# dominikbuenger/torch_nfft

Measured on AMD Instinct MI355X. Metric: Mpoints/s (adjoint+forward, 3-D N=256 m=4), higher is better.
Workload: dtype f32

## Files before the change

### torch_nfft_amd/csrc/binning.hip

```cpp
#include <algorithm>
#include <hipcub/hipcub.hpp>

#include "common.h"
#include "kernels.h"
#include "range_items.h"

namespace nfft {

constexpr int kSortBlockPoints = 8192;
constexpr int kSortThreads = 512;
constexpr int kMaxPencilsLds = 8192;
constexpr int kSort2Parts = 8;

PlanLayout plan_layout(const Geom &g, int64_t n, int64_t B)
{
    PlanLayout L;
    L.cap = g.owned ? 4 * n : n;
    L.ntiles = (int64_t)g.tiles_per_batch * B * g.SB;
    L.npencils = (int64_t)g.nta[1] * g.nta[2] * B * g.l1seg;
    L.block_points = 1024;
    while (L.block_points < kSortBlockPoints &&
           (n > L.block_points * 512 || L.npencils * ((n + L.block_points - 1) / L.block_points) > (int64_t(1) << 20)))
        L.block_points *= 2;
    L.nblocks = (n + L.block_points - 1) / L.block_points;
    L.two_level = L.npencils <= kMaxPencilsLds && L.npencils * L.nblocks < (int64_t(1) << 28) && n > 0;
    const int64_t scan_items = L.two_level ? L.npencils * L.nblocks + 1 : L.ntiles + 1;
    L.scan_bytes = align_up(scan_items / 64 + 65536, 256);
    int64_t o = 0;
    L.off_offsets = o; o = align_up(o + (L.ntiles + 1) * 4, 256);
    L.off_cursor = o;  o = align_up(o + (L.ntiles + 1) * 4, 256);
    L.off_seal = o;    o += kSealBytes;
    L.off_perm = o;    o = align_up(o + (g.dim == 3 ? 0 : L.cap * 4), 256);
    L.off_spos = o;    o = align_up(o + L.cap * g.pstride * 4, 256);
    L.off_scan = o;    o = align_up(o + L.scan_bytes, 256);
    L.off_hist = o;    o = align_up(o + (L.two_level ? scan_items * 4 : 0), 256);
    L.off_hscan = o;   o = align_up(o + (L.two_level ? scan_items * 4 : 0), 256);
    L.off_tmp = o;     o = align_up(o + (L.two_level ? L.cap * 16 : 0), 256);
    L.off_hist2 = o;   o = align_up(o + (L.two_level ? L.npencils * kSort2Parts * (int64_t)g.l1bins * g.SB * g.CG * 4 : 0), 256);
    L.grouped = L.two_level && g.CG == 3;
    L.off_groups = o;  o = align_up(o + (L.grouped ? L.ntiles * 2 * 4 : 0), 256);
    L.work_cap = g.wide ? (int64_t)g.nta[1] * g.nta[2] * B * kSegMax + L.cap / 2048 + 16 : 0;
    L.work_head = 1 + (B * 8 + 15) / 16;
    L.off_work = o;    o = align_up(o + (g.wide ? (L.work_head + 2 * L.work_cap) * 16 : 0), 256);
    L.off_sealpart = o; o = align_up(o + (L.two_level ? L.nblocks * 8 : 0), 256);
    L.off_key1 = o;    o = align_up(o + (L.two_level && !g.owned ? n * 2 : 0), 256);
    L.off_key2 = o;    o = align_up(o + (L.two_level ? L.cap * 2 : 0), 256);
    L.total = o;
    return L;
}

__device__ __forceinline__ int point_tiles(const Geom &g, const float *__restrict__ pos, const int64_t *__restrict__ batch,
                                           int64_t i, int64_t B, int tiles[4])
{
    int cell[3] = {0, 0, 0};
    for (int u = 0; u < g.dim; ++u) {
        float fr;
        split_cell(pos[i * g.dim + u], g.M, cell[u + 3 - g.dim], fr);
    }
    int64_t b = batch ? batch[i] : 0;
    b = b < 0 ? 0 : (b >= B ? B - 1 : b);
    if (g.owned) {
        int pen[4];
        const int k = owned_pencils(g, cell[1], cell[2], pen);
        for (int q = 0; q < k; ++q) tiles[q] = (int)b * g.tiles_per_batch + pen[q] * g.np0 + cell[0];
        return k;
    }
    tiles[0] = ((int)b * g.tiles_per_batch + tile_of_cells(g, cell)) * g.SB + sub_of_cells(g, cell);
    return 1;
}

constexpr int kSealThreads = 1024;
// ... 121 lines not shown
    const int64_t hi = min(n, lo + block_points);
    unsigned long long seal = 0;
    for (int64_t i0 = lo + threadIdx.x; i0 < hi; i0 += (int64_t)kSortThreads * kSortUnroll) {
        float c0[kSortUnroll], c1[kSortUnroll], c2[kSortUnroll];
        int64_t bb[kSortUnroll];
#pragma unroll
        for (int q = 0; q < kSortUnroll; ++q) {
            const int64_t i = i0 + (int64_t)q * kSortThreads;
            const bool live = i < hi;
            load_point(pos, g.dim, i, live, c0[q], c1[q], c2[q]);
            bb[q] = live && batch ? batch[i] : 0;
        }
#pragma unroll
        for (int q = 0; q < kSortUnroll; ++q) {
            if (i0 + (int64_t)q * kSortThreads >= hi) continue;
            if (seal_part) seal += seal_point(g.dim, i0 + (int64_t)q * kSortThreads, c0[q], c1[q], c2[q], batch != nullptr, bb[q]);
            if (bb[q] < 0 || bb[q] >= B) report_fault(status, kFaultBatchIndex);
            const int64_t b = bb[q] < 0 ? 0 : (bb[q] >= B ? B - 1 : bb[q]);
            int bins[4];
            const int k = l1_bins_of(g, c0[q], c1[q], c2[q], b, bins);
            for (int r = 0; r < k; ++r) atomicAdd(&lds_hist[bins[r]], 1);
            if (!g.owned) key1[i0 + (int64_t)q * kSortThreads] = (unsigned short)bins[0];
        }
    }
    __syncthreads();
    for (int i = threadIdx.x; i < npencils; i += kSortThreads) hist[(int64_t)i * nblocks + blockIdx.x] = lds_hist[i];
    if (seal_part) {
        __shared__ unsigned long long part[16];
        seal = seal_block_sum(seal, part);
        if (threadIdx.x == 0) seal_part[blockIdx.x] = seal;
    }
}

template <bool COMMON>
__global__ void __launch_bounds__(kSortThreads)
sort1_scatter_kernel(Geom g_in, const float *__restrict__ pos, const int64_t *__restrict__ batch, int64_t n, int64_t B,
                     int npencils, int nblocks, int block_points, const int *__restrict__ hscan, const unsigned short *__restrict__ key1,
                     float4 *__restrict__ tmp, const unsigned long long *__restrict__ seal_part, unsigned long long *__restrict__ seal,
                     int *__restrict__ final_offsets, int *__restrict__ final_perm, float *__restrict__ final_spos,
                     const int *__restrict__ hist_raw)
{
    const bool final_pass = !COMMON && final_offsets != nullptr;
    const bool local_scan = final_pass && hist_raw != nullptr;
    if (final_pass && !local_scan && blockIdx.x == 0) {
        for (int i = threadIdx.x; i <= npencils; i += kSortThreads) final_offsets[i] = hscan[(int64_t)i * nblocks];
    }
    if (seal && blockIdx.x == 0) {
        __shared__ unsigned long long part[16];
        unsigned long long sum = 0;
        for (int i = threadIdx.x; i < nblocks; i += kSortThreads) sum += seal_part[i];
        sum = seal_block_sum(sum, part);
        if (threadIdx.x == 0) seal[0] = sum;
        if (threadIdx.x >= 1 && threadIdx.x < (int)(kSealBytes / 8)) seal[threadIdx.x] = 0ull;
        __syncthreads();
    }
    Geom g = g_in;
    if constexpr (COMMON) { g.dim = 3; g.owned = 0; }
    extern __shared__ int lds_cur[];
    if (local_scan) {
        int *const row = lds_cur + npencils;
        for (int i = threadIdx.x; i < npencils; i += kSortThreads) { lds_cur[i] = 0; row[i] = 0; }
        __syncthreads();
        int G = 1;
        while (2 * G * npencils <= kSortThreads && G < 64) G *= 2;
        const int sub = threadIdx.x & (G - 1);
        for (int p = threadIdx.x / G; p < npencils; p += kSortThreads / G) {
            int all = 0, before = 0;
            for (int bl = sub; bl < nblocks; bl += G) {
                const int c = hist_raw[p * nblocks + bl];
                all += c;
                before += bl < (int)blockIdx.x ? c : 0;
            }
            if (all) atomicAdd(&row[p], all);
            if (before) atomicAdd(&lds_cur[p], before);
        }
        __syncthreads();
        if (threadIdx.x < 64) {
            int carry = 0;
            for (int base = 0; base < npencils; base += 64) {
                const int idx = base + threadIdx.x;
                const int tot = idx < npencils ? row[idx] : 0;
                int incl = tot;
                for (int off = 1; off < 64; off <<= 1) {
                    const int t = __shfl_up(incl, off);
                    if ((int)threadIdx.x >= off) incl += t;
                }
                if (idx < npencils) {
                    const int excl = carry + incl - tot;
                    lds_cur[idx] += excl;
                    if (blockIdx.x == 0) final_offsets[idx] = excl;
// ... 10 lines not shown
    const int64_t hi = min(n, lo + block_points);
    for (int64_t i0 = lo + threadIdx.x; i0 < hi; i0 += (int64_t)kSortThreads * kSortUnroll) {
        float c0[kSortUnroll], c1[kSortUnroll], c2[kSortUnroll];
        int64_t bb[kSortUnroll];
        int kk[kSortUnroll];
#pragma unroll
        for (int q = 0; q < kSortUnroll; ++q) {
            const int64_t i = i0 + (int64_t)q * kSortThreads;
            const bool live = i < hi;
            load_point(pos, g.dim, i, live, c0[q], c1[q], c2[q]);
            bb[q] = live && batch && g.owned ? batch[i] : 0;
            kk[q] = live && !g.owned ? key1[i] : 0;
        }
#pragma unroll
        for (int q = 0; q < kSortUnroll; ++q) {
            const int64_t i = i0 + (int64_t)q * kSortThreads;
            if (i >= hi) continue;
            int bins[4];
            int k = 1;
            if (!g.owned) {
                bins[0] = kk[q];
            } else {
                const int64_t b = bb[q] < 0 ? 0 : (bb[q] >= B ? B - 1 : bb[q]);
                k = l1_bins_of(g, c0[q], c1[q], c2[q], b, bins);
            }
            for (int r = 0; r < k; ++r) {
                const int slot = atomicAdd(&lds_cur[bins[r]], 1);
                if (final_pass) {
                    final_perm[slot] = (int)i;
                    final_spos[(int64_t)slot * g.dim] = c0[q];
                    if (g.dim > 1) final_spos[(int64_t)slot * g.dim + 1] = c1[q];
                    continue;
                }
                tmp[slot] = make_float4(c0[q], c1[q], c2[q], __int_as_float((int)i));
            }
        }
    }
}

__device__ __forceinline__ int fine_key(const Geom &g, const float4 rec, const int bin_lo, const int col0)
{
    if (g.dim != 3) return 0;
    int cell[3];
    float fr;
    split_cell(rec.x, g.M, cell[0], fr);
    int key = (g.bin0 == 1 ? cell[0] : div_small(cell[0], g.bin0)) - bin_lo;
    if (g.SB > 1) {
        split_cell(rec.y, g.M, cell[1], fr);
        split_cell(rec.z, g.M, cell[2], fr);
        key = key * g.SB + sub_of_cells(g, cell);
    }
    if (g.CG > 1) {
        split_cell(rec.z, g.M, cell[2], fr);
        key = key * g.CG + column_group(cell[2] - col0, g.W);
    }
    return key;
}

__device__ __forceinline__ void sort2_range(const int *__restrict__ hscan, int l1, int nblocks, int part, int &p0,
                                            int &r0, int &r1)
{
    p0 = hscan[(int64_t)l1 * nblocks];
    const int p1 = hscan[(int64_t)(l1 + 1) * nblocks];
    const int64_t len = p1 - p0;
    r0 = p0 + (int)(len * part / kSort2Parts);
    r1 = p0 + (int)(len * (part + 1) / kSort2Parts);
}

template <bool COMMON>
__global__ void __launch_bounds__(kSortThreads)
sort2_count_kernel(Geom g_in, int nblocks, const int *__restrict__ hscan, const float4 *__restrict__ tmp,
                   int *__restrict__ hist2 , unsigned short *__restrict__ key2 )
{
    Geom g = g_in;
    if constexpr (COMMON) { g.dim = 3; g.owned = 0; }
    extern __shared__ int lds2[];
    const int l1 = blockIdx.x, part = blockIdx.y;
    const int pencil = l1 / g.l1seg, sg = l1 - pencil * g.l1seg;
    const int bin_lo = sg * g.l1bins;
    const int col0 = (pencil % g.nta[2]) * g.Ta[2];
    const int nt0 = (min(g.np0, bin_lo + g.l1bins) - bin_lo) * g.SB * g.CG;
    int p0, r0, r1;
    sort2_range(hscan, l1, nblocks, part, p0, r0, r1);
    for (int i = threadIdx.x; i < nt0; i += kSortThreads) lds2[i] = 0;
    __syncthreads();
    for (int j0 = r0 + threadIdx.x; j0 < r1; j0 += kSortThreads * 8) {
        float4 rec[8];
#pragma unroll
        for (int q = 0; q < 8; ++q) {
            const int j = j0 + q * kSortThreads;
            rec[q] = j < r1 ? tmp[j] : make_float4(0.f, 0.f, 0.f, 0.f);
        }
#pragma unroll
        for (int q = 0; q < 8; ++q)
            if (j0 + q * kSortThreads < r1) {
                const int key = fine_key(g, rec[q], bin_lo, col0);
                atomicAdd(&lds2[key], 1);
                key2[j0 + q * kSortThreads] = (unsigned short)key;
            }
    }
    __syncthreads();
    int *out = hist2 + ((int64_t)l1 * kSort2Parts + part) * g.l1bins * g.SB * g.CG;
    for (int i = threadIdx.x; i < nt0; i += kSortThreads) out[i] = lds2[i];
}

__global__ void __launch_bounds__(kSortThreads)
sort2_scatter_kernel(Geom g, int npencils, int nblocks, const int *__restrict__ hscan, const float4 *__restrict__ tmp,
                     const int *__restrict__ hist2, const unsigned short *__restrict__ key2, int *__restrict__ offsets,
                     int *__restrict__ groups, int *__restrict__ perm, float *__restrict__ spos)
{
    extern __shared__ int lds2[];
    const int l1 = blockIdx.x, part = blockIdx.y;
    const int pencil = l1 / g.l1seg, sg = l1 - pencil * g.l1seg;
    const int bin_lo = sg * g.l1bins;
    const int nt0 = (min(g.np0, bin_lo + g.l1bins) - bin_lo) * g.SB * g.CG;
    const int64_t obase = ((int64_t)pencil * g.np0 + bin_lo) * g.SB;
    int p0, r0, r1;
    sort2_range(hscan, l1, nblocks, part, p0, r0, r1);
    const int *table = hist2 + (int64_t)l1 * kSort2Parts * g.l1bins * g.SB * g.CG;
    const int kstride = g.l1bins * g.SB * g.CG;
    int *const tot_lds = lds2 + kstride;
    for (int idx = threadIdx.x; idx < nt0; idx += kSortThreads) {
        int tot = 0, before = 0;
#pragma unroll
        for (int q = 0; q < kSort2Parts; ++q) {
            const int c = table[q * kstride + idx];
            tot += c;
            before += q < part ? c : 0;
        }
        tot_lds[idx] = tot;
        lds2[idx] = before;
    }
    __syncthreads();
    if (threadIdx.x < 64) {
        int carry = 0;
        for (int base = 0; base < nt0; base += 64) {
            const int idx = base + threadIdx.x;
            const int tot = idx < nt0 ? tot_lds[idx] : 0;
            int incl = tot;
            for (int off = 1; off < 64; off <<= 1) {
                const int t = __shfl_up(incl, off);
                if ((int)threadIdx.x >= off) incl += t;
            }
            if (idx < nt0) {
                const int excl = carry + incl - tot;
                lds2[idx] += p0 + excl;
                if (part == 0) {
                    const int bin = idx / g.CG, grp = idx - bin * g.CG;
                    if (grp == 0) offsets[obase + bin] = p0 + excl;
                    else groups[(obase + bin) * 2 + grp - 1] = p0 + excl;
                }
            }
            carry += __shfl(incl, 63);
        }
        if (part == 0 && l1 == npencils - 1 && threadIdx.x == 0) offsets[obase + nt0 / g.CG] = p0 + carry;
    }
    __syncthreads();
    for (int j0 = r0 + threadIdx.x; j0 < r1; j0 += kSortThreads * 8) {
        float4 recs[8];
        int keys[8];
#pragma unroll
        for (int q = 0; q < 8; ++q) {
            const int j = j0 + q * kSortThreads;
            recs[q] = j < r1 ? tmp[j] : make_float4(0.f, 0.f, 0.f, 0.f);
            keys[q] = j < r1 ? key2[j] : 0;
        }
#pragma unroll
        for (int q = 0; q < 8; ++q) {
            if (j0 + q * kSortThreads >= r1) continue;
            const float4 rec = recs[q];
            const int slot = atomicAdd(&lds2[keys[q]], 1);
            if (g.dim == 3) {
                ((float4 *)spos)[slot] = rec;
            } else {
                perm[slot] = __float_as_int(rec.w);
                spos[(int64_t)slot * g.dim] = rec.x;
                if (g.dim > 1) spos[(int64_t)slot * g.dim + 1] = rec.y;
            }
        }
    }
}

__global__ void __launch_bounds__(64)
segment_split_kernel(Geom g, int npl , int pencils, int runs, int target,
                     const int *__restrict__ offsets, int4 *__restrict__ work, int4 *__restrict__ list, int capacity)
{
    const int pl = blockIdx.x;
    if (pl >= npl) return;
    const int r = threadIdx.x;
    if (r >= runs) return;
    const int *off = offsets + (int64_t)pl * g.np0;
    const int seg_slabs = (g.M + runs - 1) / runs;
    const int sb = min(r * seg_slabs, g.M), se = min(sb + seg_slabs, g.M);
    const int o_sb = off[sb], pts = off[se] - o_sb;
    if (se <= sb) return;
    int pieces = (int)(((int64_t)pts + target / 2) / target);
    pieces = pieces < 1 ? 1 : (pieces > kSegPieces ? kSegPieces : pieces);
    {
        const int64_t first = (int64_t)(pl / pencils) * pencils * g.np0;
        const int64_t set_pts = offsets[first + (int64_t)pencils * g.np0] - offsets[first];
        if (pieces > 1 || (pts > 0 && (double)pts * (double)(pencils * runs) >= 1.5 * (double)set_pts))
            atomicOr(&((int *)work)[2], 1);
    }
    int prev = sb;
    for (int p = 1; p <= pieces; ++p) {
        int end = se;
        if (p < pieces) {
            const int t = o_sb + (int)((int64_t)pts * p / pieces);
            int lo = prev, hi = se;
            while (lo < hi) {
                const int mid = (lo + hi) >> 1;
                if (off[mid] >= t) hi = mid; else lo = mid + 1;
// ... 199 lines not shown
                q.y = run; run += v[k + 1];
                q.z = run; run += v[k + 2];
                q.w = run; run += v[k + 3];
                *(int4 *)(out + i0 + k) = q;
            }
        } else {
#pragma unroll
            for (int k = 0; k < IPT; ++k) {
                if (i0 + k < items) out[i0 + k] = run;
                run += v[k];
            }
        }
        __syncthreads();
        if (threadIdx.x == 1023) carry_s = run;
        __syncthreads();
    }
}

static int exclusive_scan(const int *in, int *out, int64_t items, void *scratch, int64_t scratch_bytes, hipStream_t stream)
{
    if (items <= kSmallScanItems) {
        if (items <= 4096) hipLaunchKernelGGL(small_scan_kernel<4>, dim3(1), dim3(1024), 0, stream, in, out, (int)items);
        else hipLaunchKernelGGL(small_scan_kernel<16>, dim3(1), dim3(1024), 0, stream, in, out, (int)items);
        NFFT_HIP_CHECK(hipGetLastError());
        return 0;
    }
    size_t scan_bytes = 0;
    NFFT_HIP_CHECK(hipcub::DeviceScan::ExclusiveSum(nullptr, scan_bytes, in, out, (int)items, stream));
    if ((int64_t)scan_bytes > scratch_bytes) { set_error("scan scratch too small"); return 2; }
    NFFT_HIP_CHECK(hipcub::DeviceScan::ExclusiveSum(scratch, scan_bytes, in, out, (int)items, stream));
    return 0;
}

int launch_plan_points(const Geom &g, const PlanLayout &L, const float *pos, const int64_t *batch, int64_t n, int64_t B,
                       void *plan, hipStream_t stream)
{
    char *base = (char *)plan;
    int *offsets = (int *)(base + L.off_offsets);
    int *cursor = (int *)(base + L.off_cursor);
    int *perm = (int *)(base + L.off_perm);
    float *spos = (float *)(base + L.off_spos);
    unsigned long long *const seal = (unsigned long long *)(base + L.off_seal);
    if (L.two_level) {
        int *hist = (int *)(base + L.off_hist);
        int *hscan = (int *)(base + L.off_hscan);
        float4 *tmp = (float4 *)(base + L.off_tmp);
        const int npencils = (int)L.npencils, nblocks = (int)L.nblocks;
        const int64_t items = L.npencils * L.nblocks + 1;
        const size_t lds1 = (size_t)npencils * 4;
        unsigned short *key1 = (unsigned short *)(base + L.off_key1), *key2 = (unsigned short *)(base + L.off_key2);
        const bool common = g.dim == 3 && !g.owned;
        hipLaunchKernelGGL(common ? sort1_count_kernel<true> : sort1_count_kernel<false>, dim3(nblocks), dim3(kSortThreads), lds1, stream, g, pos, batch, n, B,
                           npencils, nblocks, (int)L.block_points, hist, key1, seal ? (unsigned long long *)(base + L.off_sealpart) : nullptr,
                           device_status_block());
        const bool one_level = g.dim < 3 && g.l1seg == 1 && (int64_t)g.l1bins * g.SB * g.CG == 1 && L.ntiles == L.npencils;
        const bool local_scan = one_level && items <= 16384;
        if (!local_scan)
            if (int rc = exclusive_scan(hist, hscan, items, base + L.off_scan, L.scan_bytes, stream)) return rc;
        hipLaunchKernelGGL(common ? sort1_scatter_kernel<true> : sort1_scatter_kernel<false>, dim3(nblocks), dim3(kSortThreads),
                           local_scan ? 2 * lds1 : lds1, stream, g, pos, batch, n, B,
                           npencils, nblocks, (int)L.block_points, hscan, key1, tmp, (const unsigned long long *)(base + L.off_sealpart), seal,
                           one_level ? offsets : nullptr, perm, spos, local_scan ? hist : nullptr);
        if (one_level) {
            NFFT_HIP_CHECK(hipGetLastError());
            return 0;
        }
        int *hist2 = (int *)(base + L.off_hist2);
        const size_t lds2 = (size_t)g.l1bins * g.SB * g.CG * 4;
        hipLaunchKernelGGL(common ? sort2_count_kernel<true> : sort2_count_kernel<false>, dim3(npencils, kSort2Parts), dim3(kSortThreads), lds2, stream, g, nblocks,
                           hscan, tmp, hist2, key2);
        hipLaunchKernelGGL(sort2_scatter_kernel, dim3(npencils, kSort2Parts), dim3(kSortThreads), 2 * lds2, stream, g,
                           npencils, nblocks, hscan, tmp, hist2, key2, offsets, (int *)(base + L.off_groups), perm, spos);
        if (g.wide && launch_segment_split(g, L, n, B, offsets, (int4 *)(base + L.off_work), stream)) return 2;
        NFFT_HIP_CHECK(hipGetLastError());
        return 0;
    }
    static_assert(kSealBytes == 256, "the seal block fills one alignment unit behind the cursors");
    NFFT_HIP_CHECK(hipMemsetAsync(cursor, 0, (size_t)(L.off_seal + kSealBytes - L.off_cursor), stream));
    if (n > 0) {
        hipLaunchKernelGGL(bin_count_kernel, dim3(grid_for(n, 256)), dim3(256), 0, stream, g, pos, batch, n, B, cursor,
                           (unsigned long long *)(base + L.off_seal), device_status_block());
    }
    if (int rc = exclusive_scan(cursor, offsets, L.ntiles + 1, base + L.off_scan, L.scan_bytes, stream)) return rc;
    NFFT_HIP_CHECK(hipMemsetAsync(cursor, 0, (L.ntiles + 1) * 4, stream));
    if (n > 0) {
        hipLaunchKernelGGL(bin_fill_kernel, dim3(grid_for(n, 256)), dim3(256), 0, stream, g, pos, batch, n, B, offsets,
                           cursor, perm, spos);
    }
    if (g.wide && launch_segment_split(g, L, n, B, offsets, (int4 *)(base + L.off_work), stream)) return 2;
    NFFT_HIP_CHECK(hipGetLastError());
    return 0;
}

__global__ void __launch_bounds__(kSealThreads)
points_seal_kernel(const float *__restrict__ pos, const int64_t *__restrict__ batch, int64_t n, int dim,
                   unsigned long long *__restrict__ acc, const unsigned long long *__restrict__ expect,
                   unsigned *__restrict__ arrivals, int *__restrict__ status)
{
    unsigned long long sum = 0;
    const int64_t stride = (int64_t)gridDim.x * kSealThreads;
    int64_t i = (int64_t)blockIdx.x * kSealThreads + threadIdx.x;
    if (dim == 3 && ((uintptr_t)pos & 15) == 0 && (!batch || ((uintptr_t)batch & 15) == 0)) {
        const int64_t quads = n / 4;
        const uint4 *p4 = (const uint4 *)pos;
        const uint4 *b4 = (const uint4 *)batch;
// ... 92 lines not shown
```

### torch_nfft_amd/csrc/common.h

```cpp
#pragma once
#include <hip/hip_runtime.h>
#include <stdint.h>

#include <algorithm>
#include <atomic>
#include <string>
#include <type_traits>

namespace nfft {

void set_error(const std::string &msg);
#define NFFT_HIP_CHECK(expr)                                                                      \
    do {                                                                                          \
        hipError_t _e = (expr);                                                                   \
        if (_e != hipSuccess) {                                                                   \
            nfft::set_error(std::string(#expr) + ": " + hipGetErrorString(_e));                   \
            return 4;                                                          \
        }                                                                                         \
    } while (0)

enum DeviceFault { kFaultStreamStall = 0, kFaultBatchIndex = 1, kFaultBatchOrder = 2, kFaultStalePlan = 3, kNumFaults = 4 };
constexpr int kStatusInts = 16;
int *device_status_block();

// ... 253 lines not shown
    r = r < lo ? lo : (r > hi ? hi : r);
    const int64_t groups = (nsets > 0 ? nsets : 1) * (pencils > 0 ? pencils : 1);
    while (r < hi && groups * (r + 1) <= (ncu > 0 ? ncu : 256)) ++r;
    return (int)(r > kSegMax ? kSegMax : r);
}
inline unsigned work_list_workgroups(int64_t n, int64_t nsets, int64_t pencils, int runs, int ncu)
{
    const int64_t most = pencils * runs + n / seg_target_points(n, nsets, ncu) + 1;
    const int64_t cus = ncu > 0 ? (ncu < 1024 ? ncu : 1024) : 256;
    return (unsigned)(most < cus ? (most < 1 ? 1 : most) : cus);
}
int stream_min_item_points();
inline bool stream_items(int64_t n, int64_t nsets, int ncu, int M)
{
    if (seg_target_points(n, nsets, ncu) >= stream_min_item_points()) return true;
    const double per_set = (double)n / (double)(nsets > 0 ? nsets : 1);
    return stream_min_item_points() == 3000  && per_set >= 1.0e6 &&
           per_set >= 0.1 * (double)M * (double)M * (double)M;
}
int device_cu_count();
int current_device();
constexpr int kMaxDevices = 64;
struct DeviceOnce {
    std::atomic<bool> done[kMaxDevices];
    bool first_use();
    void mark();
};

constexpr int64_t kSealBytes = 256;
struct PlanLayout {
    int64_t cap;
    int64_t ntiles;
    int64_t npencils, nblocks, block_points;
    bool two_level;
    int64_t off_offsets, off_cursor, off_perm, off_spos, off_scan, scan_bytes;
    int64_t off_seal, off_sealpart;
    int64_t off_hist, off_hscan, off_tmp, off_hist2;
    int64_t off_groups;
    int64_t off_work, work_cap, work_head;
    int64_t off_key1, off_key2;
    bool grouped;
    int64_t total;
};
inline int64_t align_up(int64_t v, int64_t a) { return (v + a - 1) / a * a; }
PlanLayout plan_layout(const Geom &g, int64_t n, int64_t B);

inline int point_splits(const Geom &g, const PlanLayout &L, int64_t n, int64_t nplanes)
{
    const int64_t blocks = (int64_t)g.nta[1] * g.nta[2] * g.nseg;
    if (blocks <= 0 || nplanes <= 0) return 1;
    const int64_t nsets = g.tiles_per_batch > 0 ? std::max<int64_t>(1, L.ntiles / ((int64_t)g.tiles_per_batch * g.SB)) : 1;
    int64_t s = (2 * (int64_t)device_cu_count() + blocks * nplanes - 1) / (blocks * nplanes);
    s = std::min(s, n / (nsets * blocks * 128));
    return (int)std::max<int64_t>(1, std::min<int64_t>(s, 32));
}

}
```

Measured before the change: 2740.

## Stage sort scatters through LDS for coalesced writes and precompute fine keys

```diff
diff --git a/torch_nfft_amd/csrc/binning.hip b/torch_nfft_amd/csrc/binning.hip
--- a/torch_nfft_amd/csrc/binning.hip
+++ b/torch_nfft_amd/csrc/binning.hip
@@ -8,9 +8,17 @@
 namespace nfft {
 
 constexpr int kSortBlockPoints = 8192;
+constexpr int kSliceBits = 13;
+static_assert(kSortBlockPoints <= (1 << kSliceBits), "slice index must fit kSliceBits");
 constexpr int kSortThreads = 512;
 constexpr int kMaxPencilsLds = 8192;
+static_assert(kMaxPencilsLds <= (1 << (31 - kSliceBits)), "bin must fit the packed word");
 constexpr int kSort2Parts = 8;
+constexpr int kStage2Points = 4096;
+constexpr int kStageLdsBytes = 160 * 1024 - 512;
+
+inline int64_t stage1_lds_bytes(int64_t block_points, int64_t npencils) { return block_points * 16 + npencils * 8; }
+inline int64_t stage2_lds_bytes(int64_t keys) { return (int64_t)kStage2Points * 18 + keys * 12; }
 
 PlanLayout plan_layout(const Geom &g, int64_t n, int64_t B)
 {
@@ -22,6 +30,8 @@
     while (L.block_points < kSortBlockPoints &&
            (n > L.block_points * 512 || L.npencils * ((n + L.block_points - 1) / L.block_points) > (int64_t(1) << 20)))
         L.block_points *= 2;
+    if (g.dim == 3 && !g.owned && L.npencils <= kMaxPencilsLds)
+        while (L.block_points > 1024 && stage1_lds_bytes(L.block_points, L.npencils) > kStageLdsBytes / 2) L.block_points /= 2;
     L.nblocks = (n + L.block_points - 1) / L.block_points;
     L.two_level = L.npencils <= kMaxPencilsLds && L.npencils * L.nblocks < (int64_t(1) << 28) && n > 0;
     const int64_t scan_items = L.two_level ? L.npencils * L.nblocks + 1 : L.ntiles + 1;
@@ -224,30 +234,58 @@
     }
 }
 
-template <bool COMMON>
+__device__ __forceinline__ int fine_key(const Geom &g, const float4 rec, const int bin_lo, const int col0)
+{
+    if (g.dim != 3) return 0;
+    int cell[3];
+    float fr;
+    split_cell(rec.x, g.M, cell[0], fr);
+    int key = (g.bin0 == 1 ? cell[0] : div_small(cell[0], g.bin0)) - bin_lo;
+    if (g.SB > 1) {
+        split_cell(rec.y, g.M, cell[1], fr);
+        split_cell(rec.z, g.M, cell[2], fr);
+        key = key * g.SB + sub_of_cells(g, cell);
+    }
+    if (g.CG > 1) {
+        split_cell(rec.z, g.M, cell[2], fr);
+        key = key * g.CG + column_group(cell[2] - col0, g.W);
+    }
+    return key;
+}
+
+__device__ __forceinline__ int l1_fine_key(const Geom &g, const int l1, const float4 rec)
+{
+    if (g.dim != 3) return 0;
+    const int pencil = g.l1seg == 1 ? l1 : div_small(l1, g.l1seg);
+    const int col0 = (pencil - div_small(pencil, g.nta[2]) * g.nta[2]) * g.Ta[2];
+    return fine_key(g, rec, (l1 - pencil * g.l1seg) * g.l1bins, col0);
+}
+
+__device__ __forceinline__ void seal_finish(const unsigned long long *__restrict__ seal_part, int nblocks,
+                                            unsigned long long *__restrict__ seal)
+{
+    __shared__ unsigned long long part[16];
+    unsigned long long sum = 0;
+    for (int i = threadIdx.x; i < nblocks; i += kSortThreads) sum += seal_part[i];
+    sum = seal_block_sum(sum, part);
+    if (threadIdx.x == 0) seal[0] = sum;
+    if (threadIdx.x >= 1 && threadIdx.x < (int)(kSealBytes / 8)) seal[threadIdx.x] = 0ull;
+    __syncthreads();
+}
+
 __global__ void __launch_bounds__(kSortThreads)
-sort1_scatter_kernel(Geom g_in, const float *__restrict__ pos, const int64_t *__restrict__ batch, int64_t n, int64_t B,
+sort1_scatter_kernel(Geom g, const float *__restrict__ pos, const int64_t *__restrict__ batch, int64_t n, int64_t B,
                      int npencils, int nblocks, int block_points, const int *__restrict__ hscan, const unsigned short *__restrict__ key1,
-                     float4 *__restrict__ tmp, const unsigned long long *__restrict__ seal_part, unsigned long long *__restrict__ seal,
-                     int *__restrict__ final_offsets, int *__restrict__ final_perm, float *__restrict__ final_spos,
-                     const int *__restrict__ hist_raw)
-{
-    const bool final_pass = !COMMON && final_offsets != nullptr;
+                     float4 *__restrict__ tmp, unsigned short *__restrict__ key2, const unsigned long long *__restrict__ seal_part,
+                     unsigned long long *__restrict__ seal, int *__restrict__ final_offsets, int *__restrict__ final_perm,
+                     float *__restrict__ final_spos, const int *__restrict__ hist_raw)
+{
+    const bool final_pass = final_offsets != nullptr;
     const bool local_scan = final_pass && hist_raw != nullptr;
     if (final_pass && !local_scan && blockIdx.x == 0) {
         for (int i = threadIdx.x; i <= npencils; i += kSortThreads) final_offsets[i] = hscan[(int64_t)i * nblocks];
     }
-    if (seal && blockIdx.x == 0) {
-        __shared__ unsigned long long part[16];
-        unsigned long long sum = 0;
-        for (int i = threadIdx.x; i < nblocks; i += kSortThreads) sum += seal_part[i];
-        sum = seal_block_sum(sum, part);
-        if (threadIdx.x == 0) seal[0] = sum;
-        if (threadIdx.x >= 1 && threadIdx.x < (int)(kSealBytes / 8)) seal[threadIdx.x] = 0ull;
-        __syncthreads();
-    }
-    Geom g = g_in;
-    if constexpr (COMMON) { g.dim = 3; g.owned = 0; }
+    if (seal && blockIdx.x == 0) seal_finish(seal_part, nblocks, seal);
     extern __shared__ int lds_cur[];
     if (local_scan) {
         int *const row = lds_cur + npencils;
@@ -324,72 +362,121 @@
                     if (g.dim > 1) final_spos[(int64_t)slot * g.dim + 1] = c1[q];
                     continue;
                 }
-                tmp[slot] = make_float4(c0[q], c1[q], c2[q], __int_as_float((int)i));
-            }
-        }
-    }
-}
-
-__device__ __forceinline__ int fine_key(const Geom &g, const float4 rec, const int bin_lo, const int col0)
-{
-    if (g.dim != 3) return 0;
-    int cell[3];
-    float fr;
-    split_cell(rec.x, g.M, cell[0], fr);
-    int key = (g.bin0 == 1 ? cell[0] : div_small(cell[0], g.bin0)) - bin_lo;
-    if (g.SB > 1) {
-        split_cell(rec.y, g.M, cell[1], fr);
-        split_cell(rec.z, g.M, cell[2], fr);
-        key = key * g.SB + sub_of_cells(g, cell);
-    }
-    if (g.CG > 1) {
-        split_cell(rec.z, g.M, cell[2], fr);
-        key = key * g.CG + column_group(cell[2] - col0, g.W);
-    }
-    return key;
-}
-
-__device__ __forceinline__ void sort2_range(const int *__restrict__ hscan, int l1, int nblocks, int part, int &p0,
-                                            int &r0, int &r1)
+                const float4 rec = make_float4(c0[q], c1[q], c2[q], __int_as_float((int)i));
+                tmp[slot] = rec;
+                key2[slot] = (unsigned short)l1_fine_key(g, bins[r], rec);
+            }
+        }
+    }
+}
+
+__global__ void __launch_bounds__(kSortThreads)
+sort1_stage_kernel(Geom g_in, const float *__restrict__ pos, int64_t n, int npencils, int nblocks, int block_points,
+                   const int *__restrict__ hist, const int *__restrict__ hscan, const unsigned short *__restrict__ key1,
+                   float4 *__restrict__ tmp, unsigned short *__restrict__ key2, const unsigned long long *__restrict__ seal_part,
+                   unsigned long long *__restrict__ seal)
+{
+    Geom g = g_in;
+    g.dim = 3;
+    g.owned = 0;
+    if (seal && blockIdx.x == 0) seal_finish(seal_part, nblocks, seal);
+    extern __shared__ float4 lds_rec[];
+    int *const cur = (int *)(lds_rec + block_points);
+    int *const dest = cur + npencils;
+    __shared__ int wave_sum[kSortThreads / 64];
+    for (int p = threadIdx.x; p < npencils; p += kSortThreads) {
+        cur[p] = hist[(int64_t)p * nblocks + blockIdx.x];
+        dest[p] = hscan[(int64_t)p * nblocks + blockIdx.x];
+    }
+    __syncthreads();
+    {
+        const int per = (npencils + kSortThreads - 1) / kSortThreads;
+        const int a = min(npencils, (int)threadIdx.x * per), b = min(npencils, a + per);
+        const int lane = threadIdx.x & 63, wave = threadIdx.x >> 6;
+        int mine = 0;
+        for (int p = a; p < b; ++p) mine += cur[p];
+        int incl = mine;
+        for (int off = 1; off < 64; off <<= 1) {
+            const int t = __shfl_up(incl, off);
+            if (lane >= off) incl += t;
+        }
+        if (lane == 63) wave_sum[wave] = incl;
+        __syncthreads();
+        int run = incl - mine;
+        for (int w = 0; w < wave; ++w) run += wave_sum[w];
+        for (int p = a; p < b; ++p) {
+            const int c = cur[p];
+            cur[p] = run;
+            dest[p] -= run;
+            run += c;
+        }
+    }
+    __syncthreads();
+    const int64_t lo = (int64_t)blockIdx.x * block_points;
+    const int64_t hi = min(n, lo + block_points);
+    for (int64_t i0 = lo + threadIdx.x; i0 < hi; i0 += (int64_t)kSortThreads * kSortUnroll) {
+        float c0[kSortUnroll], c1[kSortUnroll], c2[kSortUnroll];
+        int kk[kSortUnroll];
+#pragma unroll
+        for (int q = 0; q < kSortUnroll; ++q) {
+            const int64_t i = i0 + (int64_t)q * kSortThreads;
+            const bool live = i < hi;
+            load_point(pos, 3, i, live, c0[q], c1[q], c2[q]);
+            kk[q] = live ? key1[i] : 0;
+        }
+#pragma unroll
+        for (int q = 0; q < kSortUnroll; ++q) {
+            const int64_t i = i0 + (int64_t)q * kSortThreads;
+            if (i >= hi) continue;
+            const int bin = kk[q];
+            const int slot = atomicAdd(&cur[bin], 1);
+            lds_rec[slot] = make_float4(c0[q], c1[q], c2[q], __int_as_float((int)(i - lo) | (bin << kSliceBits)));
+        }
+    }
+    __syncthreads();
+    const int cnt = (int)(hi - lo);
+    for (int s = threadIdx.x; s < cnt; s += kSortThreads) {
+        float4 rec = lds_rec[s];
+        const int w = __float_as_int(rec.w);
+        const int bin = w >> kSliceBits;
+        const int dst = dest[bin] + s;
+        rec.w = __int_as_float((int)(lo + (w & ((1 << kSliceBits) - 1))));
+        tmp[dst] = rec;
+        key2[dst] = (unsigned short)l1_fine_key(g, bin, rec);
+    }
+}
+
+__device__ __forceinline__ bool sort2_range(const int *__restrict__ hscan, int l1, int nblocks, int part, int &p0,
+                                            int &r0, int &r1, int &parts)
 {
     p0 = hscan[(int64_t)l1 * nblocks];
     const int p1 = hscan[(int64_t)(l1 + 1) * nblocks];
     const int64_t len = p1 - p0;
-    r0 = p0 + (int)(len * part / kSort2Parts);
-    r1 = p0 + (int)(len * (part + 1) / kSort2Parts);
-}
-
-template <bool COMMON>
+    parts = (int)min<int64_t>(kSort2Parts, max<int64_t>(1, (len + kStage2Points - 1) / kStage2Points));
+    r0 = p0 + (int)(len * part / parts);
+    r1 = p0 + (int)(len * (part + 1) / parts);
+    return part < parts;
+}
+
 __global__ void __launch_bounds__(kSortThreads)
-sort2_count_kernel(Geom g_in, int nblocks, const int *__restrict__ hscan, const float4 *__restrict__ tmp,
-                   int *__restrict__ hist2 , unsigned short *__restrict__ key2 )
-{
-    Geom g = g_in;
-    if constexpr (COMMON) { g.dim = 3; g.owned = 0; }
+sort2_count_kernel(Geom g, int nblocks, const int *__restrict__ hscan, const unsigned short *__restrict__ key2,
+                   int *__restrict__ hist2 )
+{
     extern __shared__ int lds2[];
     const int l1 = blockIdx.x, part = blockIdx.y;
-    const int pencil = l1 / g.l1seg, sg = l1 - pencil * g.l1seg;
-    const int bin_lo = sg * g.l1bins;
-    const int col0 = (pencil % g.nta[2]) * g.Ta[2];
+    const int bin_lo = (l1 % g.l1seg) * g.l1bins;
     const int nt0 = (min(g.np0, bin_lo + g.l1bins) - bin_lo) * g.SB * g.CG;
-    int p0, r0, r1;
-    sort2_range(hscan, l1, nblocks, part, p0, r0, r1);
+    int p0, r0, r1, parts;
+    if (!sort2_range(hscan, l1, nblocks, part, p0, r0, r1, parts)) return;
     for (int i = threadIdx.x; i < nt0; i += kSortThreads) lds2[i] = 0;
     __syncthreads();
     for (int j0 = r0 + threadIdx.x; j0 < r1; j0 += kSortThreads * 8) {
-        float4 rec[8];
-#pragma unroll
-        for (int q = 0; q < 8; ++q) {
-            const int j = j0 + q * kSortThreads;
-            rec[q] = j < r1 ? tmp[j] : make_float4(0.f, 0.f, 0.f, 0.f);
-        }
+        int keys[8];
+#pragma unroll
+        for (int q = 0; q < 8; ++q) keys[q] = j0 + q * kSortThreads < r1 ? key2[j0 + q * kSortThreads] : -1;
 #pragma unroll
         for (int q = 0; q < 8; ++q)
-            if (j0 + q * kSortThreads < r1) {
-                const int key = fine_key(g, rec[q], bin_lo, col0);
-                atomicAdd(&lds2[key], 1);
-                key2[j0 + q * kSortThreads] = (unsigned short)key;
-            }
+            if (keys[q] >= 0) atomicAdd(&lds2[keys[q]], 1);
     }
     __syncthreads();
     int *out = hist2 + ((int64_t)l1 * kSort2Parts + part) * g.l1bins * g.SB * g.CG;
@@ -401,34 +488,38 @@
                      const int *__restrict__ hist2, const unsigned short *__restrict__ key2, int *__restrict__ offsets,
                      int *__restrict__ groups, int *__restrict__ perm, float *__restrict__ spos)
 {
-    extern __shared__ int lds2[];
+    constexpr int kPer = kStage2Points / kSortThreads;
+    const int kstride = g.l1bins * g.SB * g.CG;
+    extern __shared__ float4 lds_rec2[];
+    unsigned short *const lds_key = (unsigned short *)(lds_rec2 + kStage2Points);
+    int *const cur = (int *)(lds_key + kStage2Points);
+    int *const lcur = cur + kstride;
+    int *const dest = lcur + kstride;
     const int l1 = blockIdx.x, part = blockIdx.y;
     const int pencil = l1 / g.l1seg, sg = l1 - pencil * g.l1seg;
     const int bin_lo = sg * g.l1bins;
     const int nt0 = (min(g.np0, bin_lo + g.l1bins) - bin_lo) * g.SB * g.CG;
     const int64_t obase = ((int64_t)pencil * g.np0 + bin_lo) * g.SB;
-    int p0, r0, r1;
-    sort2_range(hscan, l1, nblocks, part, p0, r0, r1);
-    const int *table = hist2 + (int64_t)l1 * kSort2Parts * g.l1bins * g.SB * g.CG;
-    const int kstride = g.l1bins * g.SB * g.CG;
-    int *const tot_lds = lds2 + kstride;
+    int p0, r0, r1, parts;
+    if (!sort2_range(hscan, l1, nblocks, part, p0, r0, r1, parts)) return;
+    const int *table = hist2 + (int64_t)l1 * kSort2Parts * kstride;
     for (int idx = threadIdx.x; idx < nt0; idx += kSortThreads) {
         int tot = 0, before = 0;
 #pragma unroll
         for (int q = 0; q < kSort2Parts; ++q) {
-            const int c = table[q * kstride + idx];
+            const int c = q < parts ? table[q * kstride + idx] : 0;
             tot += c;
             before += q < part ? c : 0;
         }
-        tot_lds[idx] = tot;
-        lds2[idx] = before;
+        lcur[idx] = tot;
+        cur[idx] = before;
     }
     __syncthreads();
     if (threadIdx.x < 64) {
         int carry = 0;
         for (int base = 0; base < nt0; base += 64) {
             const int idx = base + threadIdx.x;
-            const int tot = idx < nt0 ? tot_lds[idx] : 0;
+            const int tot = idx < nt0 ? lcur[idx] : 0;
             int incl = tot;
             for (int off = 1; off < 64; off <<= 1) {
                 const int t = __shfl_up(incl, off);
@@ -436,7 +527,7 @@
             }
             if (idx < nt0) {
                 const int excl = carry + incl - tot;
-                lds2[idx] += p0 + excl;
+                cur[idx] += p0 + excl;
                 if (part == 0) {
                     const int bin = idx / g.CG, grp = idx - bin * g.CG;
                     if (grp == 0) offsets[obase + bin] = p0 + excl;
@@ -447,27 +538,61 @@
         }
         if (part == 0 && l1 == npencils - 1 && threadIdx.x == 0) offsets[obase + nt0 / g.CG] = p0 + carry;
     }
-    __syncthreads();
-    for (int j0 = r0 + threadIdx.x; j0 < r1; j0 += kSortThreads * 8) {
-        float4 recs[8];
-        int keys[8];
-#pragma unroll
-        for (int q = 0; q < 8; ++q) {
-            const int j = j0 + q * kSortThreads;
-            recs[q] = j < r1 ? tmp[j] : make_float4(0.f, 0.f, 0.f, 0.f);
-            keys[q] = j < r1 ? key2[j] : 0;
-        }
-#pragma unroll
-        for (int q = 0; q < 8; ++q) {
-            if (j0 + q * kSortThreads >= r1) continue;
-            const float4 rec = recs[q];
-            const int slot = atomicAdd(&lds2[keys[q]], 1);
+    for (int c0 = r0; c0 < r1; c0 += kStage2Points) {
+        const int cnt = min(r1 - c0, kStage2Points);
+        __syncthreads();
+        for (int i = threadIdx.x; i < nt0; i += kSortThreads) lcur[i] = 0;
+        __syncthreads();
+        float4 recs[kPer];
+        int keys[kPer];
+#pragma unroll
+        for (int q = 0; q < kPer; ++q) {
+            const int j = threadIdx.x + q * kSortThreads;
+            recs[q] = j < cnt ? tmp[c0 + j] : make_float4(0.f, 0.f, 0.f, 0.f);
+            keys[q] = j < cnt ? key2[c0 + j] : -1;
+        }
+#pragma unroll
+        for (int q = 0; q < kPer; ++q)
+            if (keys[q] >= 0) atomicAdd(&lcur[keys[q]], 1);
+        __syncthreads();
+        if (threadIdx.x < 64) {
+            int carry = 0;
+            for (int base = 0; base < nt0; base += 64) {
+                const int idx = base + threadIdx.x;
+                const int c = idx < nt0 ? lcur[idx] : 0;
+                int incl = c;
+                for (int off = 1; off < 64; off <<= 1) {
+                    const int t = __shfl_up(incl, off);
+                    if ((int)threadIdx.x >= off) incl += t;
+                }
+                if (idx < nt0) {
+                    const int first = carry + incl - c;
+                    lcur[idx] = first;
+                    dest[idx] = cur[idx] - first;
+                    cur[idx] += c;
+                }
+                carry += __shfl(incl, 63);
+            }
+        }
+        __syncthreads();
+#pragma unroll
+        for (int q = 0; q < kPer; ++q) {
+            if (keys[q] < 0) continue;
+            const int slot = atomicAdd(&lcur[keys[q]], 1);
+            lds_rec2[slot] = recs[q];
+            lds_key[slot] = (unsigned short)keys[q];
+        }
+        __syncthreads();
+#pragma unroll 4
+        for (int s = threadIdx.x; s < cnt; s += kSortThreads) {
+            const float4 rec = lds_rec2[s];
+            const int dst = dest[lds_key[s]] + s;
             if (g.dim == 3) {
-                ((float4 *)spos)[slot] = rec;
+                ((float4 *)spos)[dst] = rec;
             } else {
-                perm[slot] = __float_as_int(rec.w);
-                spos[(int64_t)slot * g.dim] = rec.x;
-                if (g.dim > 1) spos[(int64_t)slot * g.dim + 1] = rec.y;
+                perm[dst] = __float_as_int(rec.w);
+                spos[(int64_t)dst * g.dim] = rec.x;
+                if (g.dim > 1) spos[(int64_t)dst * g.dim + 1] = rec.y;
             }
         }
     }
@@ -758,22 +883,41 @@
                            device_status_block());
         const bool one_level = g.dim < 3 && g.l1seg == 1 && (int64_t)g.l1bins * g.SB * g.CG == 1 && L.ntiles == L.npencils;
         const bool local_scan = one_level && items <= 16384;
+        static DeviceOnce lds_attr;
+        if (lds_attr.first_use()) {
+            NFFT_HIP_CHECK(hipFuncSetAttribute((const void *)sort1_scatter_kernel, hipFuncAttributeMaxDynamicSharedMemorySize,
+                                               2 * kMaxPencilsLds * 4));
+            NFFT_HIP_CHECK(hipFuncSetAttribute((const void *)sort1_stage_kernel, hipFuncAttributeMaxDynamicSharedMemorySize,
+                                               kStageLdsBytes));
+            NFFT_HIP_CHECK(hipFuncSetAttribute((const void *)sort2_scatter_kernel, hipFuncAttributeMaxDynamicSharedMemorySize,
+                                               kStageLdsBytes));
+            lds_attr.mark();
+        }
         if (!local_scan)
             if (int rc = exclusive_scan(hist, hscan, items, base + L.off_scan, L.scan_bytes, stream)) return rc;
-        hipLaunchKernelGGL(common ? sort1_scatter_kernel<true> : sort1_scatter_kernel<false>, dim3(nblocks), dim3(kSortThreads),
-                           local_scan ? 2 * lds1 : lds1, stream, g, pos, batch, n, B,
-                           npencils, nblocks, (int)L.block_points, hscan, key1, tmp, (const unsigned long long *)(base + L.off_sealpart), seal,
-                           one_level ? offsets : nullptr, perm, spos, local_scan ? hist : nullptr);
+        const unsigned long long *seal_part = (const unsigned long long *)(base + L.off_sealpart);
+        if (common) {
+            const int64_t lds = stage1_lds_bytes(L.block_points, npencils);
+            if (lds > kStageLdsBytes) { set_error("plan: first-level slice does not fit LDS"); return 2; }
+            hipLaunchKernelGGL(sort1_stage_kernel, dim3(nblocks), dim3(kSortThreads), (size_t)lds, stream, g, pos, n, npencils,
+                               nblocks, (int)L.block_points, hist, hscan, key1, tmp, key2, seal_part, seal);
+        } else {
+            hipLaunchKernelGGL(sort1_scatter_kernel, dim3(nblocks), dim3(kSortThreads), local_scan ? 2 * lds1 : lds1, stream, g,
+                               pos, batch, n, B, npencils, nblocks, (int)L.block_points, hscan, key1, tmp, key2, seal_part,
+                               seal, one_level ? offsets : nullptr, perm, spos, local_scan ? hist : nullptr);
+        }
         if (one_level) {
             NFFT_HIP_CHECK(hipGetLastError());
             return 0;
         }
         int *hist2 = (int *)(base + L.off_hist2);
-        const size_t lds2 = (size_t)g.l1bins * g.SB * g.CG * 4;
-        hipLaunchKernelGGL(common ? sort2_count_kernel<true> : sort2_count_kernel<false>, dim3(npencils, kSort2Parts), dim3(kSortThreads), lds2, stream, g, nblocks,
-                           hscan, tmp, hist2, key2);
-        hipLaunchKernelGGL(sort2_scatter_kernel, dim3(npencils, kSort2Parts), dim3(kSortThreads), 2 * lds2, stream, g,
-                           npencils, nblocks, hscan, tmp, hist2, key2, offsets, (int *)(base + L.off_groups), perm, spos);
+        const int64_t keys = (int64_t)g.l1bins * g.SB * g.CG;
+        if (stage2_lds_bytes(keys) > kStageLdsBytes) { set_error("plan: second-level keys do not fit LDS"); return 2; }
+        hipLaunchKernelGGL(sort2_count_kernel, dim3(npencils, kSort2Parts), dim3(kSortThreads), (size_t)keys * 4, stream, g,
+                           nblocks, hscan, key2, hist2);
+        hipLaunchKernelGGL(sort2_scatter_kernel, dim3(npencils, kSort2Parts), dim3(kSortThreads), (size_t)stage2_lds_bytes(keys),
+                           stream, g, npencils, nblocks, hscan, tmp, hist2, key2, offsets, (int *)(base + L.off_groups), perm,
+                           spos);
         if (g.wide && launch_segment_split(g, L, n, B, offsets, (int4 *)(base + L.off_work), stream)) return 2;
         NFFT_HIP_CHECK(hipGetLastError());
         return 0;
```

New measurement: 2742 (median of 4 runs). No clear change (+0.1%).

## Fuse second-level sort into single LDS-staged kernel for small pencils

Applied to the files above, without the earlier changes.

```diff
diff --git a/torch_nfft_amd/csrc/binning.hip b/torch_nfft_amd/csrc/binning.hip
--- a/torch_nfft_amd/csrc/binning.hip
+++ b/torch_nfft_amd/csrc/binning.hip
@@ -11,13 +11,27 @@
 constexpr int kSortThreads = 512;
 constexpr int kMaxPencilsLds = 8192;
 constexpr int kSort2Parts = 8;
+constexpr int kFuseThreads = 1024;
+constexpr int kFuseRecs = 16;
+constexpr int kFuseCap = kFuseThreads * kFuseRecs;
+constexpr int kFuseChunk = 8192;
+constexpr int kFuseMaxKeys = 4096;
+constexpr int kFuseLds = kFuseChunk * 16 + kFuseMaxKeys * 4;
 
 PlanLayout plan_layout(const Geom &g, int64_t n, int64_t B)
 {
     PlanLayout L;
     L.cap = g.owned ? 4 * n : n;
     L.ntiles = (int64_t)g.tiles_per_batch * B * g.SB;
-    L.npencils = (int64_t)g.nta[1] * g.nta[2] * B * g.l1seg;
+    L.l1bins = g.l1bins;
+    if (g.wide) {
+        const double per_slab = (double)n * (g.owned ? 2.0 : 1.0) / ((double)B * g.nta[1] * g.nta[2] * g.np0);
+        while (L.l1bins > 16 && per_slab * L.l1bins > 0.75 * kFuseCap &&
+               (int64_t)g.nta[1] * g.nta[2] * B * ((g.np0 + L.l1bins / 2 - 1) / (L.l1bins / 2)) <= kMaxPencilsLds)
+            L.l1bins /= 2;
+    }
+    L.l1seg = (g.np0 + L.l1bins - 1) / L.l1bins;
+    L.npencils = (int64_t)g.nta[1] * g.nta[2] * B * L.l1seg;
     L.block_points = 1024;
     while (L.block_points < kSortBlockPoints &&
            (n > L.block_points * 512 || L.npencils * ((n + L.block_points - 1) / L.block_points) > (int64_t(1) << 20)))
@@ -36,7 +50,7 @@
     L.off_hist = o;    o = align_up(o + (L.two_level ? scan_items * 4 : 0), 256);
     L.off_hscan = o;   o = align_up(o + (L.two_level ? scan_items * 4 : 0), 256);
     L.off_tmp = o;     o = align_up(o + (L.two_level ? L.cap * 16 : 0), 256);
-    L.off_hist2 = o;   o = align_up(o + (L.two_level ? L.npencils * kSort2Parts * (int64_t)g.l1bins * g.SB * g.CG * 4 : 0), 256);
+    L.off_hist2 = o;   o = align_up(o + (L.two_level ? L.npencils * kSort2Parts * (int64_t)L.l1bins * g.SB * g.CG * 4 : 0), 256);
     L.grouped = L.two_level && g.CG == 3;
     L.off_groups = o;  o = align_up(o + (L.grouped ? L.ntiles * 2 * 4 : 0), 256);
     L.work_cap = g.wide ? (int64_t)g.nta[1] * g.nta[2] * B * kSegMax + L.cap / 2048 + 16 : 0;
@@ -349,19 +363,32 @@
     return key;
 }
 
-__device__ __forceinline__ void sort2_range(const int *__restrict__ hscan, int l1, int nblocks, int part, int &p0,
-                                            int &r0, int &r1)
+__global__ void __launch_bounds__(1024) sort2_route_kernel(int npencils, int nblocks, const int *__restrict__ hscan,
+                                                           int *__restrict__ route)
+{
+    __shared__ int big;
+    if (threadIdx.x == 0) big = 0;
+    __syncthreads();
+    for (int l1 = threadIdx.x; l1 < npencils; l1 += 1024)
+        if (hscan[(int64_t)(l1 + 1) * nblocks] - hscan[(int64_t)l1 * nblocks] > kFuseCap) big = 1;
+    __syncthreads();
+    if (threadIdx.x == 0) *route = big ? 0 : 1;
+}
+
+__device__ __forceinline__ bool sort2_range(const int *__restrict__ hscan, int l1, int nblocks, int part,
+                                            const int *__restrict__ route, int &p0, int &r0, int &r1)
 {
     p0 = hscan[(int64_t)l1 * nblocks];
     const int p1 = hscan[(int64_t)(l1 + 1) * nblocks];
     const int64_t len = p1 - p0;
     r0 = p0 + (int)(len * part / kSort2Parts);
     r1 = p0 + (int)(len * (part + 1) / kSort2Parts);
+    return !(route && *route);
 }
 
 template <bool COMMON>
 __global__ void __launch_bounds__(kSortThreads)
-sort2_count_kernel(Geom g_in, int nblocks, const int *__restrict__ hscan, const float4 *__restrict__ tmp,
+sort2_count_kernel(Geom g_in, int nblocks, const int *__restrict__ route, const int *__restrict__ hscan, const float4 *__restrict__ tmp,
                    int *__restrict__ hist2 , unsigned short *__restrict__ key2 )
 {
     Geom g = g_in;
@@ -373,7 +400,7 @@
     const int col0 = (pencil % g.nta[2]) * g.Ta[2];
     const int nt0 = (min(g.np0, bin_lo + g.l1bins) - bin_lo) * g.SB * g.CG;
     int p0, r0, r1;
-    sort2_range(hscan, l1, nblocks, part, p0, r0, r1);
+    if (!sort2_range(hscan, l1, nblocks, part, route, p0, r0, r1)) return;
     for (int i = threadIdx.x; i < nt0; i += kSortThreads) lds2[i] = 0;
     __syncthreads();
     for (int j0 = r0 + threadIdx.x; j0 < r1; j0 += kSortThreads * 8) {
@@ -397,7 +424,7 @@
 }
 
 __global__ void __launch_bounds__(kSortThreads)
-sort2_scatter_kernel(Geom g, int npencils, int nblocks, const int *__restrict__ hscan, const float4 *__restrict__ tmp,
+sort2_scatter_kernel(Geom g, int npencils, int nblocks, const int *__restrict__ route, const int *__restrict__ hscan, const float4 *__restrict__ tmp,
                      const int *__restrict__ hist2, const unsigned short *__restrict__ key2, int *__restrict__ offsets,
                      int *__restrict__ groups, int *__restrict__ perm, float *__restrict__ spos)
 {
@@ -408,7 +435,7 @@
     const int nt0 = (min(g.np0, bin_lo + g.l1bins) - bin_lo) * g.SB * g.CG;
     const int64_t obase = ((int64_t)pencil * g.np0 + bin_lo) * g.SB;
     int p0, r0, r1;
-    sort2_range(hscan, l1, nblocks, part, p0, r0, r1);
+    if (!sort2_range(hscan, l1, nblocks, part, route, p0, r0, r1)) return;
     const int *table = hist2 + (int64_t)l1 * kSort2Parts * g.l1bins * g.SB * g.CG;
     const int kstride = g.l1bins * g.SB * g.CG;
     int *const tot_lds = lds2 + kstride;
@@ -470,6 +497,81 @@
                 if (g.dim > 1) spos[(int64_t)slot * g.dim + 1] = rec.y;
             }
         }
+    }
+}
+
+template <bool COMMON>
+__global__ void __launch_bounds__(kFuseThreads)
+sort2_lds_kernel(Geom g_in, int npencils, int nblocks, const int *__restrict__ route, const int *__restrict__ hscan,
+                 const float4 *__restrict__ tmp, int *__restrict__ offsets, int *__restrict__ groups, float4 *__restrict__ spos)
+{
+    if (!*route) return;
+    Geom g = g_in;
+    if constexpr (COMMON) { g.dim = 3; g.owned = 0; }
+    extern __shared__ float4 lds_rec[];
+    int *const cur = (int *)(lds_rec + kFuseChunk);
+    const int l1 = blockIdx.x;
+    const int p0 = hscan[(int64_t)l1 * nblocks];
+    const int len = hscan[(int64_t)(l1 + 1) * nblocks] - p0;
+    const int pencil = l1 / g.l1seg, sg = l1 - pencil * g.l1seg;
+    const int bin_lo = sg * g.l1bins;
+    const int col0 = (pencil % g.nta[2]) * g.Ta[2];
+    const int nt0 = (min(g.np0, bin_lo + g.l1bins) - bin_lo) * g.SB * g.CG;
+    const int64_t obase = ((int64_t)pencil * g.np0 + bin_lo) * g.SB;
+    for (int i = threadIdx.x; i < nt0; i += kFuseThreads) cur[i] = 0;
+    __syncthreads();
+    float4 rec[kFuseRecs];
+    int dst[kFuseRecs];
+#pragma unroll
+    for (int q = 0; q < kFuseRecs; ++q) {
+        const int j = q * kFuseThreads + (int)threadIdx.x;
+        rec[q] = j < len ? tmp[p0 + j] : make_float4(0.f, 0.f, 0.f, 0.f);
+    }
+#pragma unroll
+    for (int q = 0; q < kFuseRecs; ++q) {
+        const int j = q * kFuseThreads + (int)threadIdx.x;
+        dst[q] = -1;
+        if (j < len) {
+            const int key = fine_key(g, rec[q], bin_lo, col0);
+            dst[q] = key << 14 | atomicAdd(&cur[key], 1);
+        }
+    }
+    __syncthreads();
+    if (threadIdx.x < 64) {
+        int carry = 0;
+        for (int base = 0; base < nt0; base += 64) {
+            const int idx = base + threadIdx.x;
+            const int tot = idx < nt0 ? cur[idx] : 0;
+            int incl = tot;
+            for (int off = 1; off < 64; off <<= 1) {
+                const int t = __shfl_up(incl, off);
+                if ((int)threadIdx.x >= off) incl += t;
+            }
+            if (idx < nt0) {
+                const int excl = carry + incl - tot;
+                cur[idx] = excl;
+                const int bin = idx / g.CG, grp = idx - bin * g.CG;
+                if (grp == 0) offsets[obase + bin] = p0 + excl;
+                else groups[(obase + bin) * 2 + grp - 1] = p0 + excl;
+            }
+            carry += __shfl(incl, 63);
+        }
+        if (l1 == npencils - 1 && threadIdx.x == 0) offsets[obase + nt0 / g.CG] = p0 + carry;
+    }
+    __syncthreads();
+#pragma unroll
+    for (int q = 0; q < kFuseRecs; ++q)
+        if (dst[q] >= 0) dst[q] = cur[dst[q] >> 14] + (dst[q] & ((1 << 14) - 1));
+    for (int c0 = 0; c0 < len; c0 += kFuseChunk) {
+#pragma unroll
+        for (int q = 0; q < kFuseRecs; ++q) {
+            const unsigned s = (unsigned)(dst[q] - c0);
+            if (s < (unsigned)kFuseChunk) lds_rec[s] = rec[q];
+        }
+        __syncthreads();
+        const int cn = min(kFuseChunk, len - c0);
+        for (int s = threadIdx.x; s < cn; s += kFuseThreads) spos[p0 + c0 + s] = lds_rec[s];
+        __syncthreads();
     }
 }
 
@@ -735,9 +837,12 @@
     return 0;
 }
 
-int launch_plan_points(const Geom &g, const PlanLayout &L, const float *pos, const int64_t *batch, int64_t n, int64_t B,
+int launch_plan_points(const Geom &g_in, const PlanLayout &L, const float *pos, const int64_t *batch, int64_t n, int64_t B,
                        void *plan, hipStream_t stream)
 {
+    Geom g = g_in;
+    g.l1bins = L.l1bins;
+    g.l1seg = L.l1seg;
     char *base = (char *)plan;
     int *offsets = (int *)(base + L.off_offsets);
     int *cursor = (int *)(base + L.off_cursor);
@@ -757,7 +862,7 @@
                            npencils, nblocks, (int)L.block_points, hist, key1, seal ? (unsigned long long *)(base + L.off_sealpart) : nullptr,
                            device_status_block());
         const bool one_level = g.dim < 3 && g.l1seg == 1 && (int64_t)g.l1bins * g.SB * g.CG == 1 && L.ntiles == L.npencils;
-        const bool local_scan = one_level && items <= 16384;
+        const bool local_scan = one_level && items <= 16384 && 2 * lds1 + 16 * 8 <= 65536;
         if (!local_scan)
             if (int rc = exclusive_scan(hist, hscan, items, base + L.off_scan, L.scan_bytes, stream)) return rc;
         hipLaunchKernelGGL(common ? sort1_scatter_kernel<true> : sort1_scatter_kernel<false>, dim3(nblocks), dim3(kSortThreads),
@@ -770,10 +875,24 @@
         }
         int *hist2 = (int *)(base + L.off_hist2);
         const size_t lds2 = (size_t)g.l1bins * g.SB * g.CG * 4;
+        const bool fuse = g.dim == 3 && (int64_t)g.l1bins * g.SB * g.CG <= kFuseMaxKeys;
+        int *const route = fuse ? cursor : nullptr;
+        if (fuse) {
+            hipLaunchKernelGGL(sort2_route_kernel, dim3(1), dim3(1024), 0, stream, npencils, nblocks, hscan, route);
+            static DeviceOnce attr_done;
+            if (attr_done.first_use()) {
+                NFFT_HIP_CHECK(hipFuncSetAttribute((const void *)sort2_lds_kernel<true>, hipFuncAttributeMaxDynamicSharedMemorySize, kFuseLds));
+                NFFT_HIP_CHECK(hipFuncSetAttribute((const void *)sort2_lds_kernel<false>, hipFuncAttributeMaxDynamicSharedMemorySize, kFuseLds));
+                attr_done.mark();
+            }
+            hipLaunchKernelGGL(common ? sort2_lds_kernel<true> : sort2_lds_kernel<false>, dim3(npencils), dim3(kFuseThreads),
+                               (size_t)kFuseChunk * 16 + lds2, stream, g, npencils, nblocks, route, hscan, tmp, offsets,
+                               (int *)(base + L.off_groups), (float4 *)spos);
+        }
         hipLaunchKernelGGL(common ? sort2_count_kernel<true> : sort2_count_kernel<false>, dim3(npencils, kSort2Parts), dim3(kSortThreads), lds2, stream, g, nblocks,
-                           hscan, tmp, hist2, key2);
+                           route, hscan, tmp, hist2, key2);
         hipLaunchKernelGGL(sort2_scatter_kernel, dim3(npencils, kSort2Parts), dim3(kSortThreads), 2 * lds2, stream, g,
-                           npencils, nblocks, hscan, tmp, hist2, key2, offsets, (int *)(base + L.off_groups), perm, spos);
+                           npencils, nblocks, route, hscan, tmp, hist2, key2, offsets, (int *)(base + L.off_groups), perm, spos);
         if (g.wide && launch_segment_split(g, L, n, B, offsets, (int4 *)(base + L.off_work), stream)) return 2;
         NFFT_HIP_CHECK(hipGetLastError());
         return 0;
diff --git a/torch_nfft_amd/csrc/common.h b/torch_nfft_amd/csrc/common.h
--- a/torch_nfft_amd/csrc/common.h
+++ b/torch_nfft_amd/csrc/common.h
@@ -309,6 +309,7 @@
     int64_t cap;
     int64_t ntiles;
     int64_t npencils, nblocks, block_points;
+    int l1bins, l1seg;
     bool two_level;
     int64_t off_offsets, off_cursor, off_perm, off_spos, off_scan, scan_bytes;
     int64_t off_seal, off_sealpart;
```

Measured after the change: 2746 before, 2792 after, median of 6. 1.7% higher.
